# codihuston/eioku

Measured on AMD Instinct MI355X. Metric: frames/sec (scene+detect+embed) per node, higher is better.
Workload: dtype f16

## Files before the change

eioku_amd/csrc/knn.hip:

```cpp
#include "common.h"

#include <cstdlib>

#include <cfloat>

using namespace eioku;

namespace {

typedef float f32x16 __attribute__((ext_vector_type(16)));

constexpr int kQT = 32;
constexpr int kRT = 32;
constexpr int kWaves = 4;

template <int K>
struct TopK {
  float v[K];
  int id[K];
  __device__ __forceinline__ void init() {
#pragma unroll
    for (int p = 0; p < K; ++p) {
      v[p] = FLT_MAX;
      id[p] = 0x7FFFFFFF;
// ... 578 lines not shown
      }
    }
    const bool found = bi != 0x7FFFFFFFFFFFFFFFll;
    if (lane == 0) {
      D[(size_t)q * k + r] = found ? bv : FLT_MAX;
      I[(size_t)q * k + r] = found ? bi : -1;
    }
    if (found && lane == bl) {
      ++h;
      cv = nv;
      ci = ni;
      if (h + 1 < kin && ni >= 0) {
        nv = pd[base + h + 1];
        ni = pi[base + h + 1];
      } else {
        ni = -1;
      }
    }
  }
}

typedef __attribute__((address_space(3))) void lds_void_t;
typedef __attribute__((address_space(1))) const void gbl_cvoid_t;

__device__ __forceinline__ unsigned bf16_rne_bits(float f) {
  unsigned u = __float_as_uint(f);
  u += 0x7FFFu + ((u >> 16) & 1u);
  return u >> 16;
}

template <int D, int SPLIT>
__global__ __launch_bounds__(256) void k_split_planes(const float* __restrict__ x, long long n, long long first_tile,
                                                      const float* __restrict__ norms, u32x4k* __restrict__ hi,
                                                      float* __restrict__ hnorm, float* __restrict__ tmax) {
  constexpr int NS = D / 16, PU = NS * 64;
  const long long tile = first_tile + blockIdx.x / SPLIT;
  const int part = blockIdx.x % SPLIT;
  for (int o = part * (PU / SPLIT) + threadIdx.x; o < (part + 1) * (PU / SPLIT); o += 256) {
    const int s = o >> 6, h = (o >> 5) & 1, r = o & 31;
    const long long row = tile * 32 + r;
    float v[8];
    if (row < n) {
      const float4 a = *reinterpret_cast<const float4*>(x + (size_t)row * D + 16 * s + 8 * h);
      const float4 b = *reinterpret_cast<const float4*>(x + (size_t)row * D + 16 * s + 8 * h + 4);
      v[0] = a.x; v[1] = a.y; v[2] = a.z; v[3] = a.w; v[4] = b.x; v[5] = b.y; v[6] = b.z; v[7] = b.w;
    } else {
#pragma unroll
      for (int j = 0; j < 8; ++j) v[j] = 0.f;
    }
    unsigned hb[8];
#pragma unroll
    for (int j = 0; j < 8; ++j) hb[j] = bf16_rne_bits(v[j]);
    hi[(size_t)tile * PU + o] = u32x4k{hb[0] | (hb[1] << 16), hb[2] | (hb[3] << 16), hb[4] | (hb[5] << 16), hb[6] | (hb[7] << 16)};
  }
  if (hnorm && part == 0 && threadIdx.x < 64) {
    const int r = threadIdx.x & 31;
    const long long row = tile * 32 + r;
    const float nn = row < n ? norms[row] : 0.f;
    if (threadIdx.x < 32) hnorm[tile * 32 + r] = row < n ? 0.5f * nn : __builtin_inff();
    float m = nn < __builtin_inff() ? sqrtf(nn) : 0.f;
#pragma unroll
    for (int off = 16; off > 0; off >>= 1) m = fmaxf(m, __shfl_xor(m, off, 64));
    if (threadIdx.x == 0) tmax[tile] = m;
  }
}

struct ScanArgs {
  const u32x4k* xh;
  const float* hnorm;
  const float* tmax;
  const float* xmax;
  const u32x4k* qh;
  const float* qnorm;
  const float* tau;
  int tau_k;
  long long n, ntiles;
  long long tstride;
  int nq, nqt;
  unsigned* wl;
  int* wl_cnt;
  int wl_cap;
};

template <int D, int NW, int RT>
__global__ __launch_bounds__(NW * 64) void k_l2_scan(ScanArgs a) {
  constexpr int NS = D / 16, PU = NS * 64;
  constexpr int NDMA = (PU / 64 + NW - 1) / NW;
  extern __shared__ __attribute__((aligned(16))) unsigned char dyn_smem[];
  constexpr int NB = 4;
  u32x4k* qbuf = reinterpret_cast<u32x4k*>(dyn_smem);
  float* s_hc = reinterpret_cast<float*>(dyn_smem + (size_t)NB * PU * 16);
  float* s_sq = s_hc + a.nqt * 32;
  float* s_hx = s_sq + a.nqt * 32;
  int* s_cnt = reinterpret_cast<int*>(s_hx + NW * RT * 32);

  const int tid = threadIdx.x, lane = tid & 63;
  const int wave = __builtin_amdgcn_readfirstlane(tid >> 6);
  const int col = lane & 31, half = lane >> 5;

  for (int q = tid; q < a.nqt * 32; q += NW * 64) {
    float hc = __builtin_inff(), sq = 0.f;
    if (q < a.nq) {
      const float t = a.tau[(size_t)q * a.tau_k + (a.tau_k - 1)];
      const float qn = a.qnorm[q];
      const float nrm = sqrtf(qn) + a.xmax[0];
      hc = 0.5f * (qn - (t + 2e-5f * (1.0f + t) + 1e-6f * nrm * nrm));
      sq = 0.0078125f * 1.002f * sqrtf(qn);
    }
    s_hc[q] = hc;
    s_sq[q] = sq;
  }
  if (tid == 0) *s_cnt = 0;
  unsigned* const my_list = a.wl + (size_t)blockIdx.x * a.wl_cap * 2;

// ... 21 lines not shown
#pragma unroll
    for (int off = 16; off > 0; off >>= 1) m = fminf(m, __shfl_xor(m, off, 64));
    return m;
  };
  const long long my_tiles = wt < nwt ? (nwt - 1 - wt) / gridDim.x + 1 : 0;
  const int total = (int)(my_tiles * a.nqt);
  if (wt < nwt) {
#pragma unroll
    for (int i = 0; i < RT; ++i) {
      const long long t = tile_of(wt, i);
#pragma unroll
      for (int s = 0; s < NS; ++s) xh[i][s] = a.xh[(size_t)t * PU + s * 64 + lane];
      sxm[i] = a.tmax[t];
      hxmin[i] = tile_min_hx(t, i);
    }
    __builtin_amdgcn_s_waitcnt(0x0f70);
    __builtin_amdgcn_sched_barrier(0);
    stage_q(0, 0);
    if (total > 1) stage_q(1 % a.nqt, 1);
  }
  int it = 0;
  int stage_qt = 2 % a.nqt;
  for (; wt < nwt; wt += gridDim.x) {
    bool own[RT];
    long long row0[RT], tn[RT];
    const long long nwt_next = wt + gridDim.x;
    const bool more_tiles = nwt_next < nwt;
#pragma unroll
    for (int i = 0; i < RT; ++i) {
      own[i] = (wt * NW + wave) * RT + i < a.ntiles;
      row0[i] = tile_of(wt, i) * 32;
      tn[i] = more_tiles ? tile_of(nwt_next, i) : 0;
    }
    for (int qt = 0; qt < a.nqt; ++qt, ++it) {
      const bool last_qt = qt == a.nqt - 1;
      const bool meet = (it & 1) == 0;
      if (meet || qt == 0) __builtin_amdgcn_s_waitcnt(0x0f70);
      if (meet) {
        __builtin_amdgcn_s_waitcnt(0xc07f);
        asm volatile("" ::: "memory");
        __builtin_amdgcn_s_barrier();
        asm volatile("" ::: "memory");
        __builtin_amdgcn_sched_barrier(0);
#pragma unroll
        for (int e = 2; e < 4; ++e) {
          if (it + e < total) stage_q(stage_qt, (it + e) & (NB - 1));
          stage_qt = stage_qt + 1 == a.nqt ? 0 : stage_qt + 1;
        }
      }
      __builtin_amdgcn_sched_barrier(0);
      const u32x4k* qb = qbuf + (size_t)(it & (NB - 1)) * PU;
      const float hcq = s_hc[qt * 32 + col];
      const float sqq = s_sq[qt * 32 + col];
      f32x16 acc[RT];
#pragma unroll
      for (int i = 0; i < RT; ++i)
#pragma unroll
        for (int r = 0; r < 16; ++r) acc[i][r] = 0.f;
      constexpr int PF = RT == 2 ? 2 : 4;
      u32x4k bh[PF];
#pragma unroll
      for (int s = 0; s < PF; ++s) bh[s] = qb[s * 64 + lane];
#pragma unroll
      for (int s = 0; s < NS; ++s) {
        const bf16x8 ch = __builtin_bit_cast(bf16x8, bh[s % PF]);
#pragma unroll
// ... 27 lines not shown
        const int imx = max(max(max(i01, i23), i45), max(max(i67, i89), ib(15)));
        const float T = hxmin[i] + thr_q;
        if ((!(T > 0.f) || imx >= __float_as_int(T)) && own[i]) {
          const int qi = qt * 32 + col;
          int h4 = 4 * half;
          asm volatile("" : "+v"(h4));
#pragma unroll
          for (int g = 0; g < 4; ++g) {
            const float4 hx = *reinterpret_cast<const float4*>(s_hx + (wave * RT + i) * 32 + 8 * g + h4);
#pragma unroll
            for (int j = 0; j < 4; ++j) {
              const float hxr = j == 0 ? hx.x : (j == 1 ? hx.y : (j == 2 ? hx.z : hx.w));
              if (c[4 * g + j] >= hxr + thr_q) {
                const int pos = atomicAdd(s_cnt, 1);
                if (pos < a.wl_cap) {
                  my_list[2 * (size_t)pos] = (unsigned)qi;
                  my_list[2 * (size_t)pos + 1] = (unsigned)((int)row0[i] + 8 * g + j + h4);
                }
              }
            }
          }
        }
      }
      if (last_qt && more_tiles) {
#pragma unroll
        for (int i = 0; i < RT; ++i) {
          sxm[i] = a.tmax[tn[i]];
          hxmin[i] = tile_min_hx(tn[i], i);
        }
      }
    }
  }
  __syncthreads();
  if (tid == 0) a.wl_cnt[blockIdx.x] = *s_cnt;
}

__global__ __launch_bounds__(256) void k_scan_bin(const unsigned* __restrict__ wl, const int* __restrict__ wl_cnt, int wl_cap,
                                                  int* __restrict__ cand_i, int* __restrict__ cnt, int cap,
                                                  int* __restrict__ overflow) {
  int c = wl_cnt[blockIdx.x];
  if (c > wl_cap) {
    if (threadIdx.x == 0) atomicOr(overflow, 1);
    c = wl_cap;
  }
  const unsigned* list = wl + (size_t)blockIdx.x * wl_cap * 2;
  for (int i = threadIdx.x; i < c; i += 256) {
    const int qi = (int)list[2 * i], row = (int)list[2 * i + 1];
    const int pos = atomicAdd(cnt + qi, 1);
    if (pos < cap) cand_i[(size_t)qi * cap + pos] = row;
  }
}

template <int D>
__global__ __launch_bounds__(256) void k_scan_select(const float* __restrict__ db, const float* __restrict__ q,
                                                     const int* __restrict__ cand_i, const int* __restrict__ cnt, int cap, int k,
                                                     float* __restrict__ Dout, long long* __restrict__ Iout,
                                                     int* __restrict__ overflow) {
  extern __shared__ __attribute__((aligned(16))) unsigned char dyn_smem[];
  float* sd = reinterpret_cast<float*>(dyn_smem);
  int* si = reinterpret_cast<int*>(sd + cap);
  __shared__ float s_bv[4];
  __shared__ int s_bi[4];
  const int qi = blockIdx.x, tid = threadIdx.x, lane = tid & 63, wave = tid >> 6;
  int c = cnt[qi];
  if (c > cap) {
    if (tid == 0) atomicOr(overflow, 1);
    c = cap;
  }
  for (int j = tid; j < c; j += 256) si[j] = cand_i[(size_t)qi * cap + j];
  __syncthreads();
  {
    constexpr int NV = D / 128, U = 4;
    const int l32 = lane & 31, hw = tid >> 5;
    float4 qv[NV];
#pragma unroll
    for (int t = 0; t < NV; ++t) qv[t] = *reinterpret_cast<const float4*>(q + (size_t)qi * D + 128 * t + 4 * l32);
    for (int j0 = hw; j0 < c; j0 += 8 * U) {
      float4 xv[U][NV];
#pragma unroll
      for (int u = 0; u < U; ++u) {
        const int j = j0 + 8 * u;
        const int r = si[j < c ? j : j0];
#pragma unroll
        for (int t = 0; t < NV; ++t) xv[u][t] = *reinterpret_cast<const float4*>(db + (size_t)r * D + 128 * t + 4 * l32);
      }
#pragma unroll
      for (int u = 0; u < U; ++u) {
        float sum = 0.f;
#pragma unroll
        for (int t = 0; t < NV; ++t) {
          float e;
          e = qv[t].x - xv[u][t].x; sum = fmaf(e, e, sum);
          e = qv[t].y - xv[u][t].y; sum = fmaf(e, e, sum);
          e = qv[t].z - xv[u][t].z; sum = fmaf(e, e, sum);
          e = qv[t].w - xv[u][t].w; sum = fmaf(e, e, sum);
        }
#pragma unroll
        for (int off = 16; off > 0; off >>= 1) sum += __shfl_xor(sum, off, 64);
        const int j = j0 + 8 * u;
        if (l32 == 0 && j < c) sd[j] = sum;
      }
    }
  }
// ... 6 lines not shown
    for (int j = tid; j < c; j += 256) {
      const float v = sd[j];
      const int i = si[j];
      const bool after = v > lv || (v == lv && i > li);
      if (after && (v < bv || (v == bv && i < bi))) {
        bv = v;
        bi = i;
      }
    }
#pragma unroll
    for (int off = 32; off > 0; off >>= 1) {
      const float ov = __shfl_xor(bv, off, 64);
      const int oi = __shfl_xor(bi, off, 64);
      if (ov < bv || (ov == bv && oi < bi)) {
        bv = ov;
        bi = oi;
      }
    }
    if (lane == 0) {
      s_bv[wave] = bv;
      s_bi[wave] = bi;
    }
    __syncthreads();
    bv = s_bv[0];
    bi = s_bi[0];
#pragma unroll
    for (int w = 1; w < 4; ++w)
      if (s_bv[w] < bv || (s_bv[w] == bv && s_bi[w] < bi)) {
        bv = s_bv[w];
        bi = s_bi[w];
      }
    __syncthreads();
    if (tid == 0) {
      Dout[(size_t)qi * k + r] = bi == 0x7FFFFFFF ? FLT_MAX : bv;
      Iout[(size_t)qi * k + r] = bi == 0x7FFFFFFF ? -1 : (long long)bi;
    }
    lv = bv;
    li = bi;
    if (bi == 0x7FFFFFFF) lv = FLT_MAX;
  }
}

__global__ __launch_bounds__(1024) void k_sel_words(const unsigned* __restrict__ sel, const unsigned* __restrict__ live,
                                                    long long n, int nwords, unsigned* __restrict__ ew,
                                                    int* __restrict__ bcount) {
  __shared__ int s_cnt;
  if (threadIdx.x == 0) s_cnt = 0;
  __syncthreads();
  const int i = blockIdx.x * 1024 + threadIdx.x;
  unsigned w = 0;
  if (i < nwords) {
    w = sel ? sel[i] : 0xFFFFFFFFu;
    if (live) w &= live[i];
    const long long rem = n - (long long)i * 32;
    if (rem < 32) w &= (1u << (int)rem) - 1u;
    ew[i] = w;
  }
  const unsigned long long b = __ballot(w != 0);
  if ((threadIdx.x & 63) == 0 && b) atomicAdd(&s_cnt, __popcll(b));
  __syncthreads();
  if (threadIdx.x == 0) bcount[blockIdx.x] = s_cnt;
}

__global__ __launch_bounds__(1024) void k_sel_list(const unsigned* __restrict__ ew, const int* __restrict__ bcount, int nwords,
                                                   int* __restrict__ list, int* __restrict__ meta, long long ppm) {
  __shared__ int s_part[16], s_wc[16];
  const int tid = threadIdx.x, lane = tid & 63, wave = tid >> 6;
  int s = 0;
// ... 33 lines not shown
  const long long id = ids[i];
  if (id < 0 || id >= n) return;
  const unsigned bit = 1u << (int)(id & 31);
  const unsigned old = atomicAnd(live + (id >> 5), ~bit);
  if (old & bit) {
    atomicAdd(removed, 1);
    norms[id] = __builtin_inff();
    if (hnorm && id < planes_n) hnorm[id] = __builtin_inff();
  }
}

}

struct eioku_index {
  int d = 0;
  long long n = 0, cap = 0;
  float* x = nullptr;
  float* norms = nullptr;
  long long norms_cap = 0;
  bool attached = false;
  float* qbuf = nullptr; size_t qcap = 0;
  float* qnorm = nullptr; size_t qncap = 0;
  float* pd = nullptr; size_t pdcap = 0;
  int* pi = nullptr; size_t picap = 0;
  float* dout = nullptr; size_t dcap = 0;
  long long* iout = nullptr; size_t icap = 0;
  unsigned char* xh = nullptr; size_t xhcap = 0;
  float* hnorm = nullptr; size_t hncap = 0;
  float* tmax = nullptr; size_t tmcap = 0;
  float* xmax = nullptr;
  long long planes_n = 0;
  unsigned char* qh = nullptr; size_t qhcap = 0;
  unsigned* wl = nullptr; size_t wlcap = 0;
  int* wl_cnt = nullptr; size_t wlccap = 0;
  float* tau = nullptr; size_t taucap = 0;
  long long* tau_i = nullptr; size_t tauicap = 0;
  float* tau1 = nullptr; size_t tau1cap = 0;
  long long* tau1_i = nullptr; size_t tau1icap = 0;
  int* cand_i = nullptr; size_t cicap = 0;
  int* cnt = nullptr; size_t cntcap = 0;
  int scan_mode = 1;
  int scan_cap = 4096;
  long long scan_min_rows = 262144;
  long long scan_sample = 0;
  int scan_min_nq = 1;
  int scan_prescan = 32;
  int scan_rt = 2;
  unsigned* live = nullptr; size_t live_words = 0;
  int* removed_dev = nullptr;
  long long removed = 0;
  long long* idbuf = nullptr; size_t idcap = 0;
  unsigned* selbuf = nullptr; size_t selcap = 0;
  unsigned* ew = nullptr; size_t ewcap = 0;
  int* tlist = nullptr; size_t tlcap = 0;
  int* bcount = nullptr; size_t bccap = 0;
  int* meta = nullptr;
  int sel_list_ppm = 32000;
};

namespace {

template <typename T>
int grow(T** p, size_t* cap, size_t bytes) {
  if (*cap >= bytes) return EIOKU_OK;
  if (*p) {
    (void)hipDeviceSynchronize();
    (void)hipFree(*p);
    *p = nullptr;
    *cap = 0;
  }
  EIOKU_HIP_CHECK(hipMalloc((void**)p, bytes));
  *cap = bytes;
  return EIOKU_OK;
}

int norms_for(const float* x, long long n, int d, float* out, hipStream_t stream) {
  if (n == 0) return EIOKU_OK;
  long long blocks = (n * 64 + 255) / 256;
  const long long cap = (long long)num_cus() * 16;
// ... 21 lines not shown
    case 64: hipLaunchKernelGGL((k_flat_l2<K, 64, WIDE, SEL>), grid, dim3(256), 0, stream, a); break;
    case 128: hipLaunchKernelGGL((k_flat_l2<K, 128, WIDE, SEL>), grid, dim3(256), 0, stream, a); break;
    case 256: hipLaunchKernelGGL((k_flat_l2<K, 256, WIDE, SEL>), grid, dim3(256), 0, stream, a); break;
    case 384: hipLaunchKernelGGL((k_flat_l2<K, 384, WIDE, SEL>), grid, dim3(256), 0, stream, a); break;
    case 512: hipLaunchKernelGGL((k_flat_l2<K, 512, WIDE, SEL>), grid, dim3(256), 0, stream, a); break;
    default:
      set_error("dimension %d not supported (64, 128, 256, 384, 512)", d);
      return EIOKU_EINVAL;
  }
  EIOKU_LAUNCH_CHECK();
  return EIOKU_OK;
}

}

extern "C" {

int eioku_index_flat_create(int d, eioku_index** out) {
  EIOKU_REQUIRE_INIT();
  EIOKU_REQUIRE(out, "NULL out");
  EIOKU_REQUIRE(d == 64 || d == 128 || d == 256 || d == 384 || d == 512,
                "dimension %d not supported (64, 128, 256, 384, 512)", d);
  auto* ix = new eioku_index();
  ix->d = d;
  *out = ix;
  return EIOKU_OK;
}

void eioku_index_destroy(eioku_index* ix) {
  if (!ix) return;
  (void)hipDeviceSynchronize();
  if (ix->x && !ix->attached) (void)hipFree(ix->x);
  void* bufs[] = {ix->norms, ix->qbuf, ix->qnorm, ix->pd, ix->pi, ix->dout, ix->iout, ix->xh, ix->hnorm,
                  ix->tmax, ix->xmax, ix->qh, ix->wl, ix->wl_cnt, ix->tau, ix->tau_i, ix->tau1, ix->tau1_i, ix->cand_i, ix->cnt,
                  ix->live, ix->removed_dev, ix->idbuf, ix->selbuf, ix->ew, ix->tlist, ix->bcount, ix->meta};
  for (void* b : bufs)
    if (b) (void)hipFree(b);
  delete ix;
}

long long eioku_index_ntotal(const eioku_index* ix) { return ix ? ix->n : 0; }

long long eioku_index_nlive(const eioku_index* ix) { return ix ? ix->n - ix->removed : 0; }

}

namespace {

void forget_removals(eioku_index* ix) {
  if (ix->live) {
    (void)hipDeviceSynchronize();
    (void)hipFree(ix->live);
    ix->live = nullptr;
    ix->live_words = 0;
  }
  ix->removed = 0;
}

}

extern "C" {

int eioku_index_reset(eioku_index* ix) {
  EIOKU_REQUIRE(ix, "NULL index");
  forget_removals(ix);
  if (ix->attached) {
    ix->x = nullptr;
// ... 147 lines not shown
  if (prof) prof_start(EIOKU_PROF_KNN, stream);
  rc = -1;
  if (wide && K == 16 && !lbd && !sel_route) rc = launch_search_bf<16>(d, a, grid, stream);
  if (rc != -1) {
  } else if (sel_route) {
    if (sel_route == 1) {
      if (wide) rc = K == 16 ? launch_search_k<16, true, 1>(d, a, grid, stream) : launch_search_k<32, true, 1>(d, a, grid, stream);
      else rc = K == 16 ? launch_search_k<16, false, 1>(d, a, grid, stream) : launch_search_k<32, false, 1>(d, a, grid, stream);
    } else {
      if (wide) rc = K == 16 ? launch_search_k<16, true, 2>(d, a, grid, stream) : launch_search_k<32, true, 2>(d, a, grid, stream);
      else rc = K == 16 ? launch_search_k<16, false, 2>(d, a, grid, stream) : launch_search_k<32, false, 2>(d, a, grid, stream);
    }
  } else if (K == 1) rc = wide ? launch_search_k<1, true>(d, a, grid, stream) : launch_search_k<1, false>(d, a, grid, stream);
  else if (wide) rc = K == 16 ? launch_search_k<16, true>(d, a, grid, stream) : launch_search_k<32, true>(d, a, grid, stream);
  else rc = K == 16 ? launch_search_k<16, false>(d, a, grid, stream) : launch_search_k<32, false>(d, a, grid, stream);
  if (prof) prof_stop(EIOKU_PROF_KNN, stream);
  if (rc) return rc;
  if (slabs <= 64 && K > 1)
    hipLaunchKernelGGL(k_topk_merge_heads, dim3(nq), dim3(64), 0, stream, ix->pd, ix->pi, (int)slabs, K, stride, k, dD, dI, gate);
  else if (K == 1)
    hipLaunchKernelGGL((k_topk_merge<1>), dim3(nq), dim3(64), 0, stream, ix->pd, ix->pi, (const long long*)nullptr,
                       (int)slabs, nq, K, 1, (const long long*)nullptr, stride, k, dD, dI, gate);
  else if (K == 16)
    hipLaunchKernelGGL((k_topk_merge<16>), dim3(nq), dim3(64), 0, stream, ix->pd, ix->pi, (const long long*)nullptr,
                       (int)slabs, nq, K, 1, (const long long*)nullptr, stride, k, dD, dI, gate);
  else
    hipLaunchKernelGGL((k_topk_merge<32>), dim3(nq), dim3(64), 0, stream, ix->pd, ix->pi, (const long long*)nullptr,
                       (int)slabs, nq, K, 1, (const long long*)nullptr, stride, k, dD, dI, gate);
  EIOKU_LAUNCH_CHECK();
  return EIOKU_OK;
}

int split_planes(int d, const float* x, long long n, long long first_tile, long long tiles, const float* norms, void* hi,
                 float* hnorm, float* tmax, bool few_tiles, hipStream_t stream) {
  if (tiles <= 0) return EIOKU_OK;
#define EIOKU_SPLIT(D_)                                                                                                  \
  case D_:                                                                                                               \
    if (few_tiles)                                                                                                       \
      hipLaunchKernelGGL((k_split_planes<D_, 8>), dim3((unsigned)tiles * 8), dim3(256), 0, stream, x, n, first_tile, norms, \
                         (u32x4k*)hi, hnorm, tmax);                                                                      \
    else                                                                                                                 \
      hipLaunchKernelGGL((k_split_planes<D_, 1>), dim3((unsigned)tiles), dim3(256), 0, stream, x, n, first_tile, norms,   \
                         (u32x4k*)hi, hnorm, tmax);                                                                      \
    break;
  switch (d) {
    EIOKU_SPLIT(128)
    EIOKU_SPLIT(256)
    EIOKU_SPLIT(384)
    default:
      set_error("scan path: dimension %d not supported", d);
      return EIOKU_EINVAL;
  }
#undef EIOKU_SPLIT
  EIOKU_LAUNCH_CHECK();
  return EIOKU_OK;
}

template <typename T>
int grow_keep(T** p, size_t* cap, size_t bytes, size_t keep, hipStream_t stream) {
  if (*cap >= bytes) return EIOKU_OK;
  size_t want = *cap ? *cap : bytes;
  while (want < bytes) want += want / 2 + 1;
  T* np = nullptr;
  EIOKU_HIP_CHECK(hipMalloc((void**)&np, want));
  if (*p) {
    if (keep) EIOKU_HIP_CHECK(hipMemcpyAsync(np, *p, keep, hipMemcpyDeviceToDevice, stream));
    EIOKU_HIP_CHECK(hipStreamSynchronize(stream));
    (void)hipDeviceSynchronize();
    (void)hipFree(*p);
  }
  *p = np;
  *cap = want;
  return EIOKU_OK;
}

__global__ __launch_bounds__(1024) void k_max_f32(const float* __restrict__ v, long long n, float* __restrict__ out) {
// ... 2 lines not shown
  for (long long i = threadIdx.x; i < n; i += 1024) m = fmaxf(m, v[i]);
#pragma unroll
  for (int o = 32; o > 0; o >>= 1) m = fmaxf(m, __shfl_xor(m, o, 64));
  if ((threadIdx.x & 63) == 0) s_m[threadIdx.x >> 6] = m;
  __syncthreads();
  if (threadIdx.x == 0) {
    for (int w = 1; w < 16; ++w) m = fmaxf(m, s_m[w]);
    out[0] = m;
  }
}

int ensure_planes(eioku_index* ix, hipStream_t stream) {
  const int d = ix->d;
  const size_t tile_b = (size_t)d * 32 * 2;
  const long long ntiles = (ix->n + 31) / 32;
  const long long keep_tiles = ix->planes_n / 32;
  int rc = grow_keep(&ix->xh, &ix->xhcap, (size_t)ntiles * tile_b, (size_t)keep_tiles * tile_b, stream);
  if (rc) return rc;
  rc = grow_keep(&ix->hnorm, &ix->hncap, (size_t)ntiles * 32 * sizeof(float), (size_t)keep_tiles * 32 * sizeof(float), stream);
  if (rc) return rc;
  rc = grow_keep(&ix->tmax, &ix->tmcap, (size_t)ntiles * sizeof(float), (size_t)keep_tiles * sizeof(float), stream);
  if (rc) return rc;
  if (ix->planes_n != ix->n) {
    rc = split_planes(d, ix->x, ix->n, keep_tiles, ntiles - keep_tiles, ix->norms, ix->xh, ix->hnorm, ix->tmax, false, stream);
    if (rc) return rc;
    if (!ix->xmax) EIOKU_HIP_CHECK(hipMalloc((void**)&ix->xmax, sizeof(float)));
    hipLaunchKernelGGL(k_max_f32, dim3(1), dim3(1024), 0, stream, ix->tmax, ntiles, ix->xmax);
    EIOKU_LAUNCH_CHECK();
    ix->planes_n = ix->n;
  }
  return EIOKU_OK;
}

__global__ void k_tau_min(float* __restrict__ tau, const float* __restrict__ other, int nq, int k) {
  const int q = blockIdx.x * blockDim.x + threadIdx.x;
  if (q >= nq) return;
  const size_t j = (size_t)q * k + (k - 1);
  tau[j] = fminf(tau[j], other[j]);
}

template <int D>
int launch_scan(eioku_index* ix, ScanArgs& a, int rt, long long* grid_out, hipStream_t stream) {
  constexpr int PU = (D / 16) * 64;
  const int nw = rt == 2 ? 8 : 12;
  const size_t lds = (size_t)4 * PU * 16 + (size_t)a.nqt * 32 * 4 * 2 + (size_t)nw * rt * 32 * 4 + 16;
  const long long nwt = (a.ntiles + (long long)nw * rt - 1) / ((long long)nw * rt);
  long long grid = num_cus();
  if (grid > nwt) grid = nwt;
  long long wl_cap = ((64ll << 20) / 8) / grid;
  if (wl_cap > (1 << 20)) wl_cap = 1 << 20;
  if (ix->scan_cap < 256) wl_cap = ix->scan_cap;
  int rc = grow(&ix->wl, &ix->wlcap, (size_t)grid * wl_cap * 8);
  if (rc) return rc;
  rc = grow(&ix->wl_cnt, &ix->wlccap, (size_t)grid * sizeof(int));
  if (rc) return rc;
  a.wl = ix->wl;
  a.wl_cnt = ix->wl_cnt;
  a.wl_cap = (int)wl_cap;
  *grid_out = grid;
  if (rt == 2) {
    EIOKU_HIP_CHECK(hipFuncSetAttribute((const void*)k_l2_scan<D, 8, 2>, hipFuncAttributeMaxDynamicSharedMemorySize, (int)lds));
    hipLaunchKernelGGL((k_l2_scan<D, 8, 2>), dim3((unsigned)grid), dim3(8 * 64), lds, stream, a);
  } else {
    EIOKU_HIP_CHECK(hipFuncSetAttribute((const void*)k_l2_scan<D, 12, 1>, hipFuncAttributeMaxDynamicSharedMemorySize, (int)lds));
    hipLaunchKernelGGL((k_l2_scan<D, 12, 1>), dim3((unsigned)grid), dim3(12 * 64), lds, stream, a);
  }
  EIOKU_LAUNCH_CHECK();
  return EIOKU_OK;
}

template <int D>
int launch_select(const eioku_index* ix, const float* dq, int nq, int cap, int k, float* dD, long long* dI, int* overflow,
                  hipStream_t stream) {
  const size_t lds = (size_t)cap * 8;
  EIOKU_HIP_CHECK(hipFuncSetAttribute((const void*)k_scan_select<D>, hipFuncAttributeMaxDynamicSharedMemorySize, (int)lds));
  hipLaunchKernelGGL((k_scan_select<D>), dim3(nq), dim3(256), lds, stream, ix->x, dq, ix->cand_i, ix->cnt, cap, k, dD, dI,
                     overflow);
  EIOKU_LAUNCH_CHECK();
  return EIOKU_OK;
}

int scan_search(eioku_index* ix, const float* dq, int nq, int k, float* dD, long long* dI, hipStream_t stream) {
  const int d = ix->d;
  int rc = ensure_planes(ix, stream);
  if (rc) return rc;
  const int nqt = (nq + 31) / 32;
  rc = grow(&ix->qh, &ix->qhcap, (size_t)nqt * d * 32 * 2);
  if (rc) return rc;
  rc = grow(&ix->tau, &ix->taucap, (size_t)nq * k * sizeof(float));
  if (rc) return rc;
  rc = grow(&ix->tau_i, &ix->tauicap, (size_t)nq * k * sizeof(long long));
  if (rc) return rc;
  const int cap = ix->scan_cap;
  rc = grow(&ix->cand_i, &ix->cicap, (size_t)nq * cap * sizeof(int));
  if (rc) return rc;
  rc = grow(&ix->cnt, &ix->cntcap, ((size_t)nq + 1) * sizeof(int));
  if (rc) return rc;
  int* overflow = ix->cnt + nq;
  EIOKU_HIP_CHECK(hipMemsetAsync(ix->cnt, 0, ((size_t)nq + 1) * sizeof(int), stream));
  rc = split_planes(d, dq, nq, 0, nqt, nullptr, ix->qh, nullptr, nullptr, true, stream);
  if (rc) return rc;
  const long long ntiles_all = (ix->n + 31) / 32;
  int stride = ix->scan_prescan;
  if (stride > 0 && ntiles_all / stride < 64) stride = 0;
  long long sample = ix->scan_sample > 0 ? ix->scan_sample : ix->n / (stride ? 512 : 128);
  if (sample < 32768) sample = 32768;
  if (sample > 262144) sample = 262144;
  const int ygroups = (nq + 127) / 128;
  int sslabs = num_cus() / ygroups;
  if (sslabs < 1) sslabs = 1;
  long long srows = ((sample / sslabs + 127) / 128) * 128;
  if (srows < 512) srows = 512;
  while (sslabs > 1 && (long long)sslabs * srows * 2 > ix->n) --sslabs;
  rc = legacy_search(ix, dq, nq, k, nullptr, nullptr, ix->tau, ix->tau_i, nullptr, sslabs, srows, false, stream);
  if (rc) return rc;
  ScanArgs a;
  a.xh = (const u32x4k*)ix->xh;
  a.hnorm = ix->hnorm;
  a.tmax = ix->tmax;
  a.xmax = ix->xmax;
  a.qh = (const u32x4k*)ix->qh;
  a.qnorm = ix->qnorm;
  a.tau = ix->tau;
  a.tau_k = k;
  a.n = ix->n;
  a.nq = nq;
  a.nqt = nqt;
  long long sgrid = 0;
  auto scan_bin_select = [&](long long ntiles, long long tstride, float* outD, long long* outI, int* oflow, bool prof) -> int {
    a.ntiles = ntiles;
    a.tstride = tstride;
    if (prof) prof_start(EIOKU_PROF_KNN, stream);
    int r;
    switch (d) {
      case 128: r = launch_scan<128>(ix, a, ix->scan_rt, &sgrid, stream); break;
      case 256: r = launch_scan<256>(ix, a, ix->scan_rt, &sgrid, stream); break;
      default: r = launch_scan<384>(ix, a, ix->scan_rt, &sgrid, stream); break;
    }
    if (prof) prof_stop(EIOKU_PROF_KNN, stream);
    if (r) return r;
    hipLaunchKernelGGL(k_scan_bin, dim3((unsigned)sgrid), dim3(256), 0, stream, ix->wl, ix->wl_cnt, a.wl_cap, ix->cand_i,
                       ix->cnt, cap, oflow);
    EIOKU_LAUNCH_CHECK();
    switch (d) {
      case 128: return launch_select<128>(ix, dq, nq, cap, k, outD, outI, oflow, stream);
      case 256: return launch_select<256>(ix, dq, nq, cap, k, outD, outI, oflow, stream);
      default: return launch_select<384>(ix, dq, nq, cap, k, outD, outI, oflow, stream);
    }
  };
  if (stride > 0) {
    rc = grow(&ix->tau1, &ix->tau1cap, (size_t)nq * k * sizeof(float));
    if (rc) return rc;
    rc = grow(&ix->tau1_i, &ix->tau1icap, (size_t)nq * k * sizeof(long long));
    if (rc) return rc;
    rc = scan_bin_select((ntiles_all + stride - 1) / stride, stride, ix->tau1, ix->tau1_i, overflow, false);
    if (rc) return rc;
    hipLaunchKernelGGL(k_tau_min, dim3((unsigned)((nq + 255) / 256)), dim3(256), 0, stream, ix->tau, ix->tau1, nq, k);
    EIOKU_LAUNCH_CHECK();
    EIOKU_HIP_CHECK(hipMemsetAsync(ix->cnt, 0, ((size_t)nq + 1) * sizeof(int), stream));
  }
  rc = scan_bin_select(ntiles_all, 1, dD, dI, overflow, true);
  if (rc) return rc;
  return legacy_search(ix, dq, nq, k, nullptr, nullptr, dD, dI, overflow, 0, 0, false, stream);
}

int prepare_selector(eioku_index* ix, const unsigned* sel, int sel_mem, hipStream_t stream) {
  const int nwords = (int)((ix->n + 31) / 32);
  const int nblocks = (nwords + 1023) / 1024;
  int rc;
  const unsigned* dsel = sel;
  if (sel_mem == EIOKU_MEM_HOST) {
    rc = grow(&ix->selbuf, &ix->selcap, (size_t)nwords * sizeof(unsigned));
    if (rc) return rc;
    EIOKU_HIP_CHECK(hipMemcpyAsync(ix->selbuf, sel, (size_t)nwords * sizeof(unsigned), hipMemcpyHostToDevice, stream));
    dsel = ix->selbuf;
  }
  rc = grow(&ix->ew, &ix->ewcap, (size_t)nwords * sizeof(unsigned));
  if (rc) return rc;
  rc = grow(&ix->tlist, &ix->tlcap, (size_t)nwords * sizeof(int));
  if (rc) return rc;
  rc = grow(&ix->bcount, &ix->bccap, (size_t)nblocks * sizeof(int));
  if (rc) return rc;
  if (!ix->meta) EIOKU_HIP_CHECK(hipMalloc((void**)&ix->meta, 4 * sizeof(int)));
  hipLaunchKernelGGL(k_sel_words, dim3(nblocks), dim3(1024), 0, stream, dsel, (const unsigned*)ix->live, ix->n, nwords, ix->ew,
                     ix->bcount);
  EIOKU_LAUNCH_CHECK();
  hipLaunchKernelGGL(k_sel_list, dim3(nblocks), dim3(1024), 0, stream, (const unsigned*)ix->ew, (const int*)ix->bcount, nwords,
                     ix->tlist, ix->meta, (long long)ix->sel_list_ppm);
  EIOKU_LAUNCH_CHECK();
  return EIOKU_OK;
}

int search_impl(eioku_index* ix, const float* q, int nq, int k, const float* lbD, const int64_t* lbI, float* D,
                int64_t* I, int mem, void* stream_, const unsigned* sel = nullptr, int sel_mem = EIOKU_MEM_DEVICE) {
  EIOKU_REQUIRE_INIT();
  EIOKU_REQUIRE(ix && nq >= 0 && k >= 1, "bad argument");
  EIOKU_REQUIRE(k <= 32, "k=%d not supported (k <= 32)", k);
  EIOKU_REQUIRE(mem == EIOKU_MEM_HOST || mem == EIOKU_MEM_DEVICE, "bad mem flag %d", mem);
  EIOKU_REQUIRE((lbD == nullptr) == (lbI == nullptr), "lower bound needs both distances and ids");
  if (nq == 0) return EIOKU_OK;
  EIOKU_REQUIRE(q && D && I, "NULL buffer");
  EIOKU_REQUIRE(ix->n < (1ll << 31), "index too large");
  hipStream_t stream = (hipStream_t)stream_;
  const int d = ix->d;
  int rc;
  const float* dq = q;
  const float* dlbD = lbD;
  const long long* dlbI = (const long long*)lbI;
  if (mem == EIOKU_MEM_HOST) {
    const size_t qb = (((size_t)nq * d * sizeof(float)) + 255) & ~(size_t)255;
    const size_t lb = lbD ? (size_t)nq * (sizeof(float) + sizeof(long long)) + 256 : 0;
    rc = grow(&ix->qbuf, &ix->qcap, qb + lb);
    if (rc) return rc;
    EIOKU_HIP_CHECK(hipMemcpyAsync(ix->qbuf, q, (size_t)nq * d * sizeof(float), hipMemcpyHostToDevice, stream));
    dq = ix->qbuf;
    if (lbD) {
      long long* li = (long long*)((unsigned char*)ix->qbuf + qb);
      float* ld = (float*)(li + nq);
      EIOKU_HIP_CHECK(hipMemcpyAsync(li, lbI, (size_t)nq * sizeof(long long), hipMemcpyHostToDevice, stream));
      EIOKU_HIP_CHECK(hipMemcpyAsync(ld, lbD, (size_t)nq * sizeof(float), hipMemcpyHostToDevice, stream));
      dlbD = ld;
      dlbI = li;
    }
  }
  EIOKU_REQUIRE(((uintptr_t)dq & 15) == 0, "queries must be 16-byte aligned");
  rc = grow(&ix->qnorm, &ix->qncap, (size_t)nq * sizeof(float));
  if (rc) return rc;
  rc = norms_for(dq, nq, d, ix->qnorm, stream);
  if (rc) return rc;
  float* dD = D;
  long long* dI = (long long*)I;
  if (mem == EIOKU_MEM_HOST) {
    rc = grow(&ix->dout, &ix->dcap, (size_t)nq * k * sizeof(float));
    if (rc) return rc;
    rc = grow(&ix->iout, &ix->icap, (size_t)nq * k * sizeof(long long));
    if (rc) return rc;
    dD = ix->dout;
    dI = ix->iout;
  }
  const bool filtered = sel != nullptr && ix->n > 0;
  const bool scan = ix->scan_mode != 0 && !dlbD && !filtered && nq >= ix->scan_min_nq && k <= 32 &&
                    ix->n >= ix->scan_min_rows && (d == 128 || d == 256 || d == 384);
  if (filtered) {
    rc = prepare_selector(ix, sel, sel_mem, stream);
    if (rc) return rc;
    const int ppm = ix->sel_list_ppm;
    if (ppm > 0) {
      rc = legacy_search(ix, dq, nq, k, dlbD, dlbI, dD, dI, ppm >= 1000000 ? nullptr : ix->meta + 1, 0, 0, true, stream, 2);
      if (rc) return rc;
    }
    if (ppm < 1000000) {
      rc = legacy_search(ix, dq, nq, k, dlbD, dlbI, dD, dI, ppm <= 0 ? nullptr : ix->meta + 2, 0, 0, ppm <= 0, stream, 1);
      if (rc) return rc;
    }
  } else if (scan) {
    for (int q0 = 0; q0 < nq; q0 += 1024) {
      const int g = nq - q0 < 1024 ? nq - q0 : 1024;
      if (q0) {
        rc = norms_for(dq + (size_t)q0 * d, g, d, ix->qnorm, stream);
        if (rc) return rc;
      }
      rc = scan_search(ix, dq + (size_t)q0 * d, g, k, dD + (size_t)q0 * k, dI + (size_t)q0 * k, stream);
      if (rc) return rc;
    }
  } else {
    rc = legacy_search(ix, dq, nq, k, dlbD, dlbI, dD, dI, nullptr, 0, 0, true, stream);
    if (rc) return rc;
  }
  if (mem == EIOKU_MEM_HOST) {
    EIOKU_HIP_CHECK(hipMemcpyAsync(D, dD, (size_t)nq * k * sizeof(float), hipMemcpyDeviceToHost, stream));
    EIOKU_HIP_CHECK(hipMemcpyAsync(I, dI, (size_t)nq * k * sizeof(long long), hipMemcpyDeviceToHost, stream));
    EIOKU_HIP_CHECK(hipStreamSynchronize(stream));
  }
  return EIOKU_OK;
}

}

extern "C" {

int eioku_index_search(eioku_index* ix, const float* q, int nq, int k, float* D, int64_t* I, int mem,
                       void* stream_) {
  return search_impl(ix, q, nq, k, nullptr, nullptr, D, I, mem, stream_);
}

int eioku_index_search_after(eioku_index* ix, const float* q, int nq, int k, const float* after_D,
                             const int64_t* after_I, float* D, int64_t* I, int mem, void* stream_) {
  EIOKU_REQUIRE(after_D && after_I, "NULL lower bound");
  return search_impl(ix, q, nq, k, after_D, after_I, D, I, mem, stream_);
}

int eioku_index_search_sel(eioku_index* ix, const float* q, int nq, int k, const uint32_t* sel_words, int sel_mem,
                           const float* after_D, const int64_t* after_I, float* D, int64_t* I, int mem, void* stream_) {
  EIOKU_REQUIRE(!sel_words || sel_mem == EIOKU_MEM_HOST || sel_mem == EIOKU_MEM_DEVICE, "bad selector mem flag %d", sel_mem);
// ... 25 lines not shown
  hipLaunchKernelGGL(k_remove_ids, dim3((unsigned)((n_ids + 255) / 256)), dim3(256), 0, stream, dids, n_ids, ix->n,
                     ix->planes_n, ix->live, ix->norms, ix->hnorm, ix->removed_dev);
  EIOKU_LAUNCH_CHECK();
  int now = 0;
  EIOKU_HIP_CHECK(hipMemcpyAsync(&now, ix->removed_dev, sizeof(int), hipMemcpyDeviceToHost, stream));
  EIOKU_HIP_CHECK(hipStreamSynchronize(stream));
  ix->removed += now;
  return EIOKU_OK;
}

int eioku_index_set_param(eioku_index* ix, const char* name, long long value) {
  EIOKU_REQUIRE(ix && name, "bad argument");
  if (!strcmp(name, "sel_list_ppm")) {
    EIOKU_REQUIRE(value >= 0 && value <= 1000000, "sel_list_ppm must be in [0, 1000000] (0: never the tile list, 1000000: always)");
    ix->sel_list_ppm = (int)value;
  } else if (!strcmp(name, "scan_mode")) {
    EIOKU_REQUIRE(value == 0 || value == 1, "scan_mode is 0 (register-tile kernels only) or 1 (scan path for wide searches)");
    ix->scan_mode = (int)value;
  } else if (!strcmp(name, "scan_cap")) {
    EIOKU_REQUIRE(value >= 16 && value <= 16384, "scan_cap must be in [16, 16384]");
    ix->scan_cap = (int)value;
  } else if (!strcmp(name, "scan_min_rows")) {
    EIOKU_REQUIRE(value >= 4096, "scan_min_rows must be >= 4096");
    ix->scan_min_rows = value;
  } else if (!strcmp(name, "scan_sample")) {
    EIOKU_REQUIRE(value >= 0, "scan_sample must be >= 0");
    ix->scan_sample = value;
  } else if (!strcmp(name, "scan_min_nq")) {
    EIOKU_REQUIRE(value >= 1, "scan_min_nq must be >= 1");
    ix->scan_min_nq = (int)value;
  } else if (!strcmp(name, "scan_prescan")) {
    EIOKU_REQUIRE(value == 0 || (value >= 2 && value <= 1024), "scan_prescan is 0 (off) or a tile stride in [2, 1024]");
    ix->scan_prescan = (int)value;
  } else if (!strcmp(name, "scan_rt")) {
    EIOKU_REQUIRE(value == 1 || value == 2, "scan_rt must be 1 or 2");
    ix->scan_rt = (int)value;
  } else {
    set_error("unknown index parameter '%s'", name);
    return EIOKU_EINVAL;
  }
  return EIOKU_OK;
}

int eioku_topk_merge_ex(const float* d_lists, const int64_t* i_lists, int nlists, int nq, int k_in, int k, float* D,
                        int64_t* I, void* stream_) {
  EIOKU_REQUIRE_INIT();
  EIOKU_REQUIRE(nlists >= 1 && nq >= 0 && k >= 1 && k <= 32 && k_in >= k, "bad argument");
  if (nq == 0) return EIOKU_OK;
  EIOKU_REQUIRE(d_lists && i_lists && D && I, "NULL buffer");
  hipStream_t stream = (hipStream_t)stream_;
  if (k <= 16)
    hipLaunchKernelGGL((k_topk_merge<16>), dim3(nq), dim3(64), 0, stream, d_lists, (const int*)nullptr,
                       (const long long*)i_lists, nlists, nq, k_in, 0, (const long long*)nullptr, 0ll, k, D, (long long*)I);
  else
    hipLaunchKernelGGL((k_topk_merge<32>), dim3(nq), dim3(64), 0, stream, d_lists, (const int*)nullptr,
                       (const long long*)i_lists, nlists, nq, k_in, 0, (const long long*)nullptr, 0ll, k, D, (long long*)I);
  EIOKU_LAUNCH_CHECK();
  return EIOKU_OK;
}

int eioku_topk_merge(const float* d_lists, const int64_t* i_lists, int nlists, int nq, int k, float* D,
                     int64_t* I, void* stream_) {
  return eioku_topk_merge_ex(d_lists, i_lists, nlists, nq, k, k, D, I, stream_);
}

}
// ... 1 lines not shown
```

Before: 48050.

## Fuse scan binning into scan kernel, fold tau min and query norms, add cascade

The separate binning kernel is removed; each scan block now scatters its own worklist entries into per-query candidate lists at the end of the scan kernel. The select kernel resets the counts and takes the min into tau itself, which removes the k_tau_min kernel, a memset and the tau1 buffers. Query norms are computed inside the query plane-split kernel instead of in a separate norms pass. A scan_levels cascade knob is added that, when enabled, shrinks the initial sampled legacy search to small slabs and relies on strided prescans to seed tau, which changes the threshold quality and so how many candidates the full scan passes on.

```diff
diff --git a/eioku_amd/csrc/knn.hip b/eioku_amd/csrc/knn.hip
--- a/eioku_amd/csrc/knn.hip
+++ b/eioku_amd/csrc/knn.hip
@@ -634,10 +634,29 @@
 template <int D, int SPLIT>
 __global__ __launch_bounds__(256) void k_split_planes(const float* __restrict__ x, long long n, long long first_tile,
                                                       const float* __restrict__ norms, u32x4k* __restrict__ hi,
-                                                      float* __restrict__ hnorm, float* __restrict__ tmax) {
+                                                      float* __restrict__ hnorm, float* __restrict__ tmax,
+                                                      float* __restrict__ norms_out) {
   constexpr int NS = D / 16, PU = NS * 64;
   const long long tile = first_tile + blockIdx.x / SPLIT;
   const int part = blockIdx.x % SPLIT;
+  if (norms_out) {
+    const int lane = threadIdx.x & 63;
+    for (int r = part * (32 / SPLIT) + (threadIdx.x >> 6); r < (part + 1) * (32 / SPLIT); r += 4) {
+      const long long row = tile * 32 + r;
+      if (row >= n) break;
+      float s = 0.f;
+      for (int c = lane * 4; c < D; c += 256) {
+        const float4 v = *reinterpret_cast<const float4*>(x + (size_t)row * D + c);
+        s += v.x * v.x;
+        s += v.y * v.y;
+        s += v.z * v.z;
+        s += v.w * v.w;
+      }
+#pragma unroll
+      for (int off = 32; off > 0; off >>= 1) s += __shfl_xor(s, off, 64);
+      if (lane == 0) norms_out[row] = s;
+    }
+  }
   for (int o = part * (PU / SPLIT) + threadIdx.x; o < (part + 1) * (PU / SPLIT); o += 256) {
     const int s = o >> 6, h = (o >> 5) & 1, r = o & 31;
     const long long row = tile * 32 + r;
@@ -680,8 +699,11 @@
   long long tstride;
   int nq, nqt;
   unsigned* wl;
-  int* wl_cnt;
   int wl_cap;
+  int* cand_i;
+  int* cnt;
+  int cap;
+  int* overflow;
 };
 
 template <int D, int NW, int RT>
@@ -769,6 +791,7 @@
       row0[i] = tile_of(wt, i) * 32;
       tn[i] = more_tiles ? tile_of(nwt_next, i) : 0;
     }
+#pragma unroll 1
     for (int qt = 0; qt < a.nqt; ++qt, ++it) {
       const bool last_qt = qt == a.nqt - 1;
       const bool meet = (it & 1) == 0;
@@ -862,30 +885,24 @@
     }
   }
   __syncthreads();
-  if (tid == 0) a.wl_cnt[blockIdx.x] = *s_cnt;
-}
-
-__global__ __launch_bounds__(256) void k_scan_bin(const unsigned* __restrict__ wl, const int* __restrict__ wl_cnt, int wl_cap,
-                                                  int* __restrict__ cand_i, int* __restrict__ cnt, int cap,
-                                                  int* __restrict__ overflow) {
-  int c = wl_cnt[blockIdx.x];
-  if (c > wl_cap) {
-    if (threadIdx.x == 0) atomicOr(overflow, 1);
-    c = wl_cap;
-  }
-  const unsigned* list = wl + (size_t)blockIdx.x * wl_cap * 2;
-  for (int i = threadIdx.x; i < c; i += 256) {
-    const int qi = (int)list[2 * i], row = (int)list[2 * i + 1];
-    const int pos = atomicAdd(cnt + qi, 1);
-    if (pos < cap) cand_i[(size_t)qi * cap + pos] = row;
+  int c = *s_cnt;
+  if (c > a.wl_cap) {
+    if (tid == 0) atomicOr(a.overflow, 1);
+    c = a.wl_cap;
+  }
+  for (int i = tid; i < c; i += NW * 64) {
+    const uint2 e = *reinterpret_cast<const uint2*>(my_list + 2 * (size_t)i);
+    const int qi = (int)e.x;
+    const int pos = atomicAdd(a.cnt + qi, 1);
+    if (pos < a.cap) a.cand_i[(size_t)qi * a.cap + pos] = (int)e.y;
   }
 }
 
 template <int D>
 __global__ __launch_bounds__(256) void k_scan_select(const float* __restrict__ db, const float* __restrict__ q,
-                                                     const int* __restrict__ cand_i, const int* __restrict__ cnt, int cap, int k,
+                                                     const int* __restrict__ cand_i, int* __restrict__ cnt, int cap, int k,
                                                      float* __restrict__ Dout, long long* __restrict__ Iout,
-                                                     int* __restrict__ overflow) {
+                                                     float* __restrict__ tau, int* __restrict__ overflow) {
   extern __shared__ __attribute__((aligned(16))) unsigned char dyn_smem[];
   float* sd = reinterpret_cast<float*>(dyn_smem);
   int* si = reinterpret_cast<int*>(sd + cap);
@@ -899,6 +916,7 @@
   }
   for (int j = tid; j < c; j += 256) si[j] = cand_i[(size_t)qi * cap + j];
   __syncthreads();
+  if (tid == 0) cnt[qi] = 0;
   {
     constexpr int NV = D / 128, U = 4;
     const int l32 = lane & 31, hw = tid >> 5;
@@ -971,8 +989,12 @@
       }
     __syncthreads();
     if (tid == 0) {
-      Dout[(size_t)qi * k + r] = bi == 0x7FFFFFFF ? FLT_MAX : bv;
-      Iout[(size_t)qi * k + r] = bi == 0x7FFFFFFF ? -1 : (long long)bi;
+      const float dv = bi == 0x7FFFFFFF ? FLT_MAX : bv;
+      if (Dout) {
+        Dout[(size_t)qi * k + r] = dv;
+        Iout[(size_t)qi * k + r] = bi == 0x7FFFFFFF ? -1 : (long long)bi;
+      }
+      if (tau && r == k - 1) tau[(size_t)qi * k + r] = fminf(tau[(size_t)qi * k + r], dv);
     }
     lv = bv;
     li = bi;
@@ -1072,11 +1094,8 @@
   long long planes_n = 0;
   unsigned char* qh = nullptr; size_t qhcap = 0;
   unsigned* wl = nullptr; size_t wlcap = 0;
-  int* wl_cnt = nullptr; size_t wlccap = 0;
   float* tau = nullptr; size_t taucap = 0;
   long long* tau_i = nullptr; size_t tauicap = 0;
-  float* tau1 = nullptr; size_t tau1cap = 0;
-  long long* tau1_i = nullptr; size_t tau1icap = 0;
   int* cand_i = nullptr; size_t cicap = 0;
   int* cnt = nullptr; size_t cntcap = 0;
   int scan_mode = 1;
@@ -1085,6 +1104,7 @@
   long long scan_sample = 0;
   int scan_min_nq = 1;
   int scan_prescan = 32;
+  int scan_levels = 1;
   int scan_rt = 2;
   unsigned* live = nullptr; size_t live_words = 0;
   int* removed_dev = nullptr;
@@ -1172,7 +1192,7 @@
   (void)hipDeviceSynchronize();
   if (ix->x && !ix->attached) (void)hipFree(ix->x);
   void* bufs[] = {ix->norms, ix->qbuf, ix->qnorm, ix->pd, ix->pi, ix->dout, ix->iout, ix->xh, ix->hnorm,
-                  ix->tmax, ix->xmax, ix->qh, ix->wl, ix->wl_cnt, ix->tau, ix->tau_i, ix->tau1, ix->tau1_i, ix->cand_i, ix->cnt,
+                  ix->tmax, ix->xmax, ix->qh, ix->wl, ix->tau, ix->tau_i, ix->cand_i, ix->cnt,
                   ix->live, ix->removed_dev, ix->idbuf, ix->selbuf, ix->ew, ix->tlist, ix->bcount, ix->meta};
   for (void* b : bufs)
     if (b) (void)hipFree(b);
@@ -1386,16 +1406,16 @@
 }
 
 int split_planes(int d, const float* x, long long n, long long first_tile, long long tiles, const float* norms, void* hi,
-                 float* hnorm, float* tmax, bool few_tiles, hipStream_t stream) {
+                 float* hnorm, float* tmax, bool few_tiles, hipStream_t stream, float* norms_out = nullptr) {
   if (tiles <= 0) return EIOKU_OK;
 #define EIOKU_SPLIT(D_)                                                                                                  \
   case D_:                                                                                                               \
     if (few_tiles)                                                                                                       \
       hipLaunchKernelGGL((k_split_planes<D_, 8>), dim3((unsigned)tiles * 8), dim3(256), 0, stream, x, n, first_tile, norms, \
-                         (u32x4k*)hi, hnorm, tmax);                                                                      \
+                         (u32x4k*)hi, hnorm, tmax, norms_out);                                                           \
     else                                                                                                                 \
       hipLaunchKernelGGL((k_split_planes<D_, 1>), dim3((unsigned)tiles), dim3(256), 0, stream, x, n, first_tile, norms,   \
-                         (u32x4k*)hi, hnorm, tmax);                                                                      \
+                         (u32x4k*)hi, hnorm, tmax, norms_out);                                                           \
     break;
   switch (d) {
     EIOKU_SPLIT(128)
@@ -1464,15 +1484,8 @@
   return EIOKU_OK;
 }
 
-__global__ void k_tau_min(float* __restrict__ tau, const float* __restrict__ other, int nq, int k) {
-  const int q = blockIdx.x * blockDim.x + threadIdx.x;
-  if (q >= nq) return;
-  const size_t j = (size_t)q * k + (k - 1);
-  tau[j] = fminf(tau[j], other[j]);
-}
-
 template <int D>
-int launch_scan(eioku_index* ix, ScanArgs& a, int rt, long long* grid_out, hipStream_t stream) {
+int launch_scan(eioku_index* ix, ScanArgs& a, int rt, hipStream_t stream) {
   constexpr int PU = (D / 16) * 64;
   const int nw = rt == 2 ? 8 : 12;
   const size_t lds = (size_t)4 * PU * 16 + (size_t)a.nqt * 32 * 4 * 2 + (size_t)nw * rt * 32 * 4 + 16;
@@ -1484,12 +1497,8 @@
   if (ix->scan_cap < 256) wl_cap = ix->scan_cap;
   int rc = grow(&ix->wl, &ix->wlcap, (size_t)grid * wl_cap * 8);
   if (rc) return rc;
-  rc = grow(&ix->wl_cnt, &ix->wlccap, (size_t)grid * sizeof(int));
-  if (rc) return rc;
   a.wl = ix->wl;
-  a.wl_cnt = ix->wl_cnt;
   a.wl_cap = (int)wl_cap;
-  *grid_out = grid;
   if (rt == 2) {
     EIOKU_HIP_CHECK(hipFuncSetAttribute((const void*)k_l2_scan<D, 8, 2>, hipFuncAttributeMaxDynamicSharedMemorySize, (int)lds));
     hipLaunchKernelGGL((k_l2_scan<D, 8, 2>), dim3((unsigned)grid), dim3(8 * 64), lds, stream, a);
@@ -1502,12 +1511,12 @@
 }
 
 template <int D>
-int launch_select(const eioku_index* ix, const float* dq, int nq, int cap, int k, float* dD, long long* dI, int* overflow,
-                  hipStream_t stream) {
+int launch_select(const eioku_index* ix, const float* dq, int nq, int cap, int k, float* dD, long long* dI, float* tau,
+                  int* overflow, hipStream_t stream) {
   const size_t lds = (size_t)cap * 8;
   EIOKU_HIP_CHECK(hipFuncSetAttribute((const void*)k_scan_select<D>, hipFuncAttributeMaxDynamicSharedMemorySize, (int)lds));
   hipLaunchKernelGGL((k_scan_select<D>), dim3(nq), dim3(256), lds, stream, ix->x, dq, ix->cand_i, ix->cnt, cap, k, dD, dI,
-                     overflow);
+                     tau, overflow);
   EIOKU_LAUNCH_CHECK();
   return EIOKU_OK;
 }
@@ -1526,23 +1535,29 @@
   const int cap = ix->scan_cap;
   rc = grow(&ix->cand_i, &ix->cicap, (size_t)nq * cap * sizeof(int));
   if (rc) return rc;
-  rc = grow(&ix->cnt, &ix->cntcap, ((size_t)nq + 1) * sizeof(int));
+  rc = grow(&ix->cnt, &ix->cntcap, ((size_t)nq + 2) * sizeof(int));
   if (rc) return rc;
   int* overflow = ix->cnt + nq;
-  EIOKU_HIP_CHECK(hipMemsetAsync(ix->cnt, 0, ((size_t)nq + 1) * sizeof(int), stream));
-  rc = split_planes(d, dq, nq, 0, nqt, nullptr, ix->qh, nullptr, nullptr, true, stream);
+  int* level_overflow = ix->cnt + nq + 1;
+  EIOKU_HIP_CHECK(hipMemsetAsync(ix->cnt, 0, ((size_t)nq + 2) * sizeof(int), stream));
+  rc = split_planes(d, dq, nq, 0, nqt, nullptr, ix->qh, nullptr, nullptr, true, stream, ix->qnorm);
   if (rc) return rc;
   const long long ntiles_all = (ix->n + 31) / 32;
   int stride = ix->scan_prescan;
   if (stride > 0 && ntiles_all / stride < 64) stride = 0;
-  long long sample = ix->scan_sample > 0 ? ix->scan_sample : ix->n / (stride ? 512 : 128);
-  if (sample < 32768) sample = 32768;
-  if (sample > 262144) sample = 262144;
+  const bool cascade = stride > 0 && ix->scan_levels >= 1;
   const int ygroups = (nq + 127) / 128;
   int sslabs = num_cus() / ygroups;
   if (sslabs < 1) sslabs = 1;
-  long long srows = ((sample / sslabs + 127) / 128) * 128;
-  if (srows < 512) srows = 512;
+  long long srows = 512;
+  if (cascade && sslabs > 64) sslabs = 64;
+  if (!cascade || ix->scan_sample > 0) {
+    long long sample = ix->scan_sample > 0 ? ix->scan_sample : ix->n / (stride ? 512 : 128);
+    if (sample < 32768 && !cascade) sample = 32768;
+    if (sample > 262144) sample = 262144;
+    srows = ((sample / sslabs + 127) / 128) * 128;
+    if (srows < 512) srows = 512;
+  }
   while (sslabs > 1 && (long long)sslabs * srows * 2 > ix->n) --sslabs;
   rc = legacy_search(ix, dq, nq, k, nullptr, nullptr, ix->tau, ix->tau_i, nullptr, sslabs, srows, false, stream);
   if (rc) return rc;
@@ -1558,40 +1573,39 @@
   a.n = ix->n;
   a.nq = nq;
   a.nqt = nqt;
-  long long sgrid = 0;
-  auto scan_bin_select = [&](long long ntiles, long long tstride, float* outD, long long* outI, int* oflow, bool prof) -> int {
+  a.cand_i = ix->cand_i;
+  a.cnt = ix->cnt;
+  a.cap = cap;
+  auto scan_select = [&](long long ntiles, long long tstride, float* outD, long long* outI, int* oflow, bool prof) -> int {
     a.ntiles = ntiles;
     a.tstride = tstride;
+    a.overflow = oflow;
+    float* tau = outD ? nullptr : ix->tau;
     if (prof) prof_start(EIOKU_PROF_KNN, stream);
     int r;
     switch (d) {
-      case 128: r = launch_scan<128>(ix, a, ix->scan_rt, &sgrid, stream); break;
-      case 256: r = launch_scan<256>(ix, a, ix->scan_rt, &sgrid, stream); break;
-      default: r = launch_scan<384>(ix, a, ix->scan_rt, &sgrid, stream); break;
+      case 128: r = launch_scan<128>(ix, a, ix->scan_rt, stream); break;
+      case 256: r = launch_scan<256>(ix, a, ix->scan_rt, stream); break;
+      default: r = launch_scan<384>(ix, a, ix->scan_rt, stream); break;
     }
     if (prof) prof_stop(EIOKU_PROF_KNN, stream);
     if (r) return r;
-    hipLaunchKernelGGL(k_scan_bin, dim3((unsigned)sgrid), dim3(256), 0, stream, ix->wl, ix->wl_cnt, a.wl_cap, ix->cand_i,
-                       ix->cnt, cap, oflow);
-    EIOKU_LAUNCH_CHECK();
     switch (d) {
-      case 128: return launch_select<128>(ix, dq, nq, cap, k, outD, outI, oflow, stream);
-      case 256: return launch_select<256>(ix, dq, nq, cap, k, outD, outI, oflow, stream);
-      default: return launch_select<384>(ix, dq, nq, cap, k, outD, outI, oflow, stream);
+      case 128: return launch_select<128>(ix, dq, nq, cap, k, outD, outI, tau, oflow, stream);
+      case 256: return launch_select<256>(ix, dq, nq, cap, k, outD, outI, tau, oflow, stream);
+      default: return launch_select<384>(ix, dq, nq, cap, k, outD, outI, tau, oflow, stream);
     }
   };
   if (stride > 0) {
-    rc = grow(&ix->tau1, &ix->tau1cap, (size_t)nq * k * sizeof(float));
-    if (rc) return rc;
-    rc = grow(&ix->tau1_i, &ix->tau1icap, (size_t)nq * k * sizeof(long long));
-    if (rc) return rc;
-    rc = scan_bin_select((ntiles_all + stride - 1) / stride, stride, ix->tau1, ix->tau1_i, overflow, false);
-    if (rc) return rc;
-    hipLaunchKernelGGL(k_tau_min, dim3((unsigned)((nq + 255) / 256)), dim3(256), 0, stream, ix->tau, ix->tau1, nq, k);
-    EIOKU_LAUNCH_CHECK();
-    EIOKU_HIP_CHECK(hipMemsetAsync(ix->cnt, 0, ((size_t)nq + 1) * sizeof(int), stream));
-  }
-  rc = scan_bin_select(ntiles_all, 1, dD, dI, overflow, true);
+    for (int lv = (cascade ? ix->scan_levels : 1) - 1; lv >= 0; --lv) {
+      long long s = stride;
+      for (int j = 0; j < lv && s <= ntiles_all; ++j) s *= 4;
+      if (ntiles_all / s < 64) continue;
+      rc = scan_select((ntiles_all + s - 1) / s, s, nullptr, nullptr, level_overflow, false);
+      if (rc) return rc;
+    }
+  }
+  rc = scan_select(ntiles_all, 1, dD, dI, overflow, true);
   if (rc) return rc;
   return legacy_search(ix, dq, nq, k, nullptr, nullptr, dD, dI, overflow, 0, 0, false, stream);
 }
@@ -1658,8 +1672,6 @@
   EIOKU_REQUIRE(((uintptr_t)dq & 15) == 0, "queries must be 16-byte aligned");
   rc = grow(&ix->qnorm, &ix->qncap, (size_t)nq * sizeof(float));
   if (rc) return rc;
-  rc = norms_for(dq, nq, d, ix->qnorm, stream);
-  if (rc) return rc;
   float* dD = D;
   long long* dI = (long long*)I;
   if (mem == EIOKU_MEM_HOST) {
@@ -1673,6 +1685,10 @@
   const bool filtered = sel != nullptr && ix->n > 0;
   const bool scan = ix->scan_mode != 0 && !dlbD && !filtered && nq >= ix->scan_min_nq && k <= 32 &&
                     ix->n >= ix->scan_min_rows && (d == 128 || d == 256 || d == 384);
+  if (!scan) {
+    rc = norms_for(dq, nq, d, ix->qnorm, stream);
+    if (rc) return rc;
+  }
   if (filtered) {
     rc = prepare_selector(ix, sel, sel_mem, stream);
     if (rc) return rc;
@@ -1688,10 +1704,6 @@
   } else if (scan) {
     for (int q0 = 0; q0 < nq; q0 += 1024) {
       const int g = nq - q0 < 1024 ? nq - q0 : 1024;
-      if (q0) {
-        rc = norms_for(dq + (size_t)q0 * d, g, d, ix->qnorm, stream);
-        if (rc) return rc;
-      }
       rc = scan_search(ix, dq + (size_t)q0 * d, g, k, dD + (size_t)q0 * k, dI + (size_t)q0 * k, stream);
       if (rc) return rc;
     }
@@ -1783,6 +1795,9 @@
   } else if (!strcmp(name, "scan_prescan")) {
     EIOKU_REQUIRE(value == 0 || (value >= 2 && value <= 1024), "scan_prescan is 0 (off) or a tile stride in [2, 1024]");
     ix->scan_prescan = (int)value;
+  } else if (!strcmp(name, "scan_levels")) {
+    EIOKU_REQUIRE(value >= 0 && value <= 8, "scan_levels is 0 (sample + one pre-scan) or the number of cascade levels in [1, 8]");
+    ix->scan_levels = (int)value;
   } else if (!strcmp(name, "scan_rt")) {
     EIOKU_REQUIRE(value == 1 || value == 2, "scan_rt must be 1 or 2");
     ix->scan_rt = (int)value;
```

New measurement: 47860. Within noise of the previous version (-0.4%).
